# anonymousauthors001/SGS-GNN

Measured on AMD Instinct MI355X. Metric: sampled edges/sec + training steps/sec, Reddit hybrid 20% sparsity, higher is better.
Workload: dtype f32

## Files before the change

include/sgs_hip.h:

```cpp
#ifndef SGS_HIP_H_
#define SGS_HIP_H_

#include <stddef.h>
#include <stdint.h>

#ifdef __cplusplus
extern "C" {
#endif

#define SGS_ABI_VERSION 1

#define SGS_OK 0
#define SGS_EINVAL (-1)
#define SGS_EWORKSPACE (-2)
#define SGS_EHIP (-3)

typedef void* sgs_stream_t;

int sgs_abi_version(void);
const char* sgs_last_error(void);

int sgs_rng_set_epoch_buffer(const uint64_t* epoch_dev);
int sgs_exp_noise(uint64_t seed, uint64_t stream_id, int64_t E, float* noise, sgs_stream_t stream);
int sgs_dropout_keep(uint64_t seed, uint32_t site, int64_t rows, int64_t cols, float p, uint8_t* keep,
// ... 102 lines not shown
                          float* Hn, sgs_stream_t stream);
int sgs_gcn_norm_bwd_edge(const float* gw_hat, const float* gloop, int64_t n_edges, int64_t N, const float* dis,
                          const int32_t* loop_eid, const int64_t* edge_index, const float* Hn, float* dw,
                          sgs_stream_t stream);

#define SGS_ACT_NONE 0
#define SGS_ACT_RELU 1
#define SGS_ACT_RELU_DROPOUT 2
int sgs_spmm_csr(const float* X, int64_t N, int64_t D, int64_t nnz, const int32_t* ptr, const int32_t* col, const float* val,
                 const float* diag, const float* bias, int act, float p_drop, uint64_t seed, uint32_t site, float* Y,
                 sgs_stream_t stream);

int sgs_sddmm_csr(const float* A, const float* B, int64_t N, int64_t D, int64_t nnz, const int32_t* ptr, const int32_t* col,
                  const int32_t* eid, float* g, float* gdiag, sgs_stream_t stream);

int sgs_spmm_csr_variant(int64_t N, int64_t D, int64_t nnz, int aligned16);
int sgs_sddmm_csr_variant(int64_t N, int64_t D, int64_t nnz, int aligned16);

int sgs_act_bwd(const float* dY, const float* Y, int64_t n, int act, float p_drop, float* dZ, sgs_stream_t stream);
size_t sgs_colsum_workspace_bytes(int64_t N, int64_t D);
int sgs_colsum(const float* A, int64_t N, int64_t D, float* out, void* ws, size_t ws_bytes, sgs_stream_t stream);
int sgs_act_bwd_colsum(const float* dY, const float* Y, int64_t N, int64_t D, int act, float p_drop, float* dZ, float* colsum, void* ws,
                       size_t ws_bytes, sgs_stream_t stream);

int sgs_colsum_variant(int64_t N, int64_t D, int fused_act);

int sgs_gcn_pair_ok(int64_t N, int64_t nnz, int64_t D);
int sgs_spmm_csr_next(const float* X, int64_t N, int64_t D, int64_t nnz, const int32_t* ptr, const int32_t* col, const float* val,
                      const float* diag, const float* bias, int act, float p_drop, uint64_t seed, uint32_t site, const float* Wn, int64_t Dn,
                      float* Y, float* Z, sgs_stream_t stream);
int sgs_spmm_csr_bwd_prev(const float* dZ, int64_t N, int64_t D, int64_t nnz, const int32_t* ptr, const int32_t* col, const float* val,
                          const float* diag, const float* W, int64_t Dp, const float* Yp, int act, float p_drop, float* dX, float* dZp,
                          float* colsum, sgs_stream_t stream);

size_t sgs_edge_score_workspace_bytes(int64_t N, int64_t H, int64_t E);
int sgs_edge_score_hidden_supported(int64_t H);
int sgs_edge_score_get_variant(void);
int sgs_edge_score_get_bwd_variant(void);
void sgs_edge_score_set_bwd_variant(int variant);
int sgs_edge_score_bwd_tile(void);
void sgs_edge_score_set_variant(int variant);
int sgs_edge_score_fwd(const float* codes, const float* U, int64_t N, int64_t H, const int64_t* edge_index, int64_t E,
                       int64_t edge_id_offset, const float* W1, const float* b1, const float* w2, const float* b2,
                       float p_drop, uint64_t seed, uint32_t site, float* p_out, void* ws, size_t ws_bytes,
                       sgs_stream_t stream);
size_t sgs_edge_mates_workspace_bytes(int64_t n_edges);
int sgs_edge_mates(const int64_t* edge_index, int64_t n_edges, int64_t N, const int32_t* out_ptr, const int32_t* out_dst,
                   const int32_t* out_eid, int32_t* mate, void* ws, size_t ws_bytes, sgs_stream_t stream);
int sgs_edge_score_paired_supported(int64_t H);
int sgs_edge_score_fwd_paired(const float* codes, const float* U, int64_t N, int64_t H, const int64_t* edge_index, int64_t E,
                              int64_t edge_id_offset, const int32_t* canon, int64_t M, const int32_t* mate, const float* W1, const float* b1,
                              const float* w2, const float* b2, float p_drop, uint64_t seed, uint32_t site, float* p_out, void* ws,
                              size_t ws_bytes, sgs_stream_t stream);
int sgs_edge_score_bwd_core(const float* codes, const float* U, int64_t N, int64_t H, const int64_t* edge_index,
                            int64_t E, int64_t edge_id_offset, const int64_t* active_eid, int64_t n_active, const float* grad_p,
                            const float* W1, const float* b1, const float* w2, const float* b2, float p_drop,
                            uint64_t seed, uint32_t site, float* dv, float* hdz_part, float* dz, float* feat, void* ws,
                            size_t ws_bytes, sgs_stream_t stream);
int sgs_edge_score_bwd_dfeat_supported(int64_t H);
int sgs_edge_score_bwd_dfeat(const float* dv, int64_t n, int64_t H, const float* W1, float* dfeat, void* ws, size_t ws_bytes,
                             sgs_stream_t stream);

int sgs_edge_score_bwd_bits_supported(int64_t H);
int sgs_edge_score_fwd_mask(const float* codes, const float* U, int64_t N, int64_t H, const int64_t* edge_index, int64_t E,
                            int64_t edge_id_offset, const int32_t* canon, int64_t M, const int32_t* mate, const float* W1, const float* b1,
                            const float* w2, const float* b2, float p_drop, uint64_t seed, uint32_t site, float* p_out, uint32_t* maskbits,
// ... 316 lines not shown
```

sgs-gnn_amd/csrc/gcn.hip:

```cpp
#include "sgs_common.h"

namespace sgs {
size_t graph_sort_workspace_bytes(int64_t n, int64_t N);
size_t graph_src_sorted_workspace_bytes(int64_t n, int64_t N);
int graph_build_src_sorted(const int64_t* ei, int64_t n, int64_t N, int32_t* in_ptr, int32_t* in_src, int32_t* in_eid, int32_t* out_ptr,
                           int32_t* out_dst, int32_t* out_eid, int32_t* loop_eid, int32_t* unsorted_flag, void* ws, size_t ws_bytes,
                           hipStream_t stream);
int graph_build_by_sort(const int64_t* ei, int64_t n, int64_t N, int32_t* in_ptr, int32_t* in_src, int32_t* in_eid, int32_t* out_ptr,
                        int32_t* out_dst, int32_t* out_eid, int32_t* loop_eid, void* ws, size_t ws_bytes, hipStream_t stream);
}

namespace sgs {
namespace {

constexpr int kT = 256;
constexpr int kMaxLdsRow = 8192;

__global__ void __launch_bounds__(kT) count_degrees(const int64_t* __restrict__ ei, int64_t n_edges, int* __restrict__ cnt_in,
                                                   int* __restrict__ cnt_out, int* __restrict__ loop_eid) {
    const int64_t e = static_cast<int64_t>(blockIdx.x) * kT + threadIdx.x;
    if (e >= n_edges) return;
    const int s = static_cast<int>(ei[e]), d = static_cast<int>(ei[n_edges + e]);
    atomicAdd(&cnt_in[d], 1);
    atomicAdd(&cnt_out[s], 1);
// ... 968 lines not shown
                                                                 const float* __restrict__ val, const float* __restrict__ diag,
                                                                 const float* __restrict__ bias, int act, float* __restrict__ Y) {
    const int64_t d = blockIdx.y;
    spmm_csr_rowblock_body<VEC, NW>(X + d * xs, N, D, ptr + d * (N + 1), col + d * nnz, val + d * nnz, diag ? diag + d * N : nullptr, bias, act,
                                    1.0f, 0u, uint64_t(0), 0u, nullptr, Y + d * N * D);
}

enum { kPairCol = 0, kPairFwd = 1, kPairBwd = 2 };
constexpr int kPairMaxD = 512;
constexpr int kPairWlds = 12288;
constexpr int kPairWpre = kPairWlds / 1024;
template <class FY, class FW>
__device__ __forceinline__ float lib_gemm_dot(int K, FY y, FW w) {
    const int Kmain = K / 16 * 16;
    float z = 0.f;
    if (Kmain > 0) {
        float ya[8], wa[8];
#pragma unroll
        for (int u = 0; u < 8; ++u) { const int k = 2 * (u & 3) + (u >> 2); ya[u] = y(k); wa[u] = w(k); }
        for (int b = 0; b < Kmain; b += 8) {
            const int nb = b + 8 < Kmain ? b + 8 : b;
            float yn[8], wn[8];
#pragma unroll
            for (int u = 0; u < 8; ++u) { const int k = nb + 2 * (u & 3) + (u >> 2); yn[u] = y(k); wn[u] = w(k); }
#pragma unroll
            for (int u = 0; u < 8; ++u) z = fmaf(ya[u], wa[u], z);
#pragma unroll
            for (int u = 0; u < 8; ++u) { ya[u] = yn[u]; wa[u] = wn[u]; }
        }
    }
    for (int k = Kmain; k < K; ++k) z = fmaf(y(k), w(k), z);
    return z;
}
template <int VEC, int NW, int MODE>
__global__ void __launch_bounds__(1024) spmm_rowgroup_pair(const float* __restrict__ X, int64_t N, int64_t D, const int* __restrict__ ptr,
                                                           const int* __restrict__ col, const float* __restrict__ val,
                                                           const float* __restrict__ diag, const float* __restrict__ bias, int act,
                                                           float drop_scale, uint32_t drop_thresh, uint64_t seed, uint32_t site,
                                                           const uint64_t* __restrict__ epoch, float* __restrict__ Y,
                                                           const float* __restrict__ Wn, int64_t Dn, const float* __restrict__ Yp,
                                                           float* __restrict__ Zn, int ncs, float* __restrict__ colsum) {
    using V = typename VecT<VEC>::type;
    constexpr int RG = 16 / NW;
    __shared__ float part[RG][NW][64 * VEC];
    __shared__ __align__(16) float ys[RG * kPairMaxD];
    __shared__ float wl[MODE == kPairFwd ? kPairWlds : 1];
    if (MODE != kPairFwd && static_cast<int>(blockIdx.x) < ncs) {
        if (D % 4 == 0) colsum_small_v4_body<false>(X, nullptr, N, D, SGS_ACT_NONE, 1.f, nullptr, colsum, blockIdx.x);
        else            colsum_small_body<false>(X, nullptr, N, D, SGS_ACT_NONE, 1.f, nullptr, colsum, blockIdx.x);
        return;
    }
    seed = fold_epoch(seed, epoch);
    const int lane = threadIdx.x & 63, wave = (threadIdx.x >> 6) % NW, grp = threadIdx.x / (64 * NW);
    const int64_t row0 = static_cast<int64_t>(blockIdx.x - ncs) * RG;
    const int64_t i = row0 + grp;
    const bool live = i < N;
    int b = 0, e = 0;
    float dg = 0.f;
    uint32_t rkey = 0;
    const int yact = MODE == kPairBwd ? SGS_ACT_NONE : act;
    if (live) {
        b = ptr[i];
        e = ptr[i + 1];
        dg = diag ? diag[i] : 0.f;
        rkey = dropout_row_key(seed, site, static_cast<uint64_t>(i));
    }
    const bool wlds = MODE == kPairFwd && Dn * D <= kPairWlds;
    float wpre[MODE == kPairFwd ? kPairWpre : 1];
    if (MODE == kPairFwd && wlds) {
#pragma unroll
        for (int u = 0; u < kPairWpre; ++u) {
            const int64_t idx = threadIdx.x + 1024 * u;
            wpre[u] = idx < Dn * D ? Wn[idx] : 0.f;
        }
    }
    for (int64_t cbase = 0; cbase < D; cbase += 64 * VEC) {
        const int64_t c0 = cbase + static_cast<int64_t>(lane) * VEC;
        const bool in = c0 < D;
        float acc[VEC];
#pragma unroll
        for (int v = 0; v < VEC; ++v) acc[v] = 0.f;
        if (in) {
            int k = b + wave;
            for (; k + 7 * NW < e; k += 8 * NW) {
                int j[8]; float w[8]; V x[8];
#pragma unroll
                for (int u = 0; u < 8; ++u) { j[u] = col[k + NW * u]; w[u] = val[k + NW * u]; }
#pragma unroll
                for (int u = 0; u < 8; ++u) x[u] = *reinterpret_cast<const V*>(X + static_cast<int64_t>(j[u]) * D + c0);
#pragma unroll
                for (int u = 0; u < 8; ++u) {
                    float xv[VEC];
                    *reinterpret_cast<V*>(xv) = x[u];
#pragma unroll
                    for (int v = 0; v < VEC; ++v) acc[v] = fmaf(w[u], xv[v], acc[v]);
                }
            }
            for (; k < e; k += NW) {
                float xv[VEC];
                *reinterpret_cast<V*>(xv) = *reinterpret_cast<const V*>(X + static_cast<int64_t>(col[k]) * D + c0);
                const float w = val[k];
#pragma unroll
                for (int v = 0; v < VEC; ++v) acc[v] = fmaf(w, xv[v], acc[v]);
            }
        }
#pragma unroll
        for (int v = 0; v < VEC; ++v) part[grp][wave][lane * VEC + v] = acc[v];
        __syncthreads();
        const int t = threadIdx.x % (64 * NW);
        if (live && t < 64 * VEC && cbase + t < D) {
            const int64_t c = cbase + t;
            float y = 0.f;
#pragma unroll
            for (int g = 0; g < NW; g += 4) y += (part[grp][g][t] + part[grp][g + 1][t]) + (part[grp][g + 2][t] + part[grp][g + 3][t]);
            if (diag) y = fmaf(dg, X[i * D + c], y);
            if (bias) y += bias[c];
            if (yact != SGS_ACT_NONE) y = fmaxf(y, 0.f);
            if (yact == SGS_ACT_RELU_DROPOUT) y = dropout_keep_col(rkey, static_cast<uint32_t>(c), drop_thresh) ? y * drop_scale : 0.f;
            Y[i * D + c] = y;
            ys[grp * D + c] = y;
        }
        __syncthreads();
    }
    if (MODE == kPairFwd) {
        if (wlds) {
#pragma unroll
            for (int u = 0; u < kPairWpre; ++u) {
                const int64_t idx = threadIdx.x + 1024 * u;
                if (idx < Dn * D) {
                    const int64_t o = idx / D, k = idx - o * D;
                    wl[k * Dn + o] = wpre[u];
                }
            }
            __syncthreads();
        }
        for (int64_t idx = threadIdx.x; idx < RG * Dn; idx += 1024) {
            const int r = static_cast<int>(idx / Dn);
            const int64_t o = idx - r * Dn, ir = row0 + r;
            if (ir >= N) break;
            const float* yr = ys + r * D;
            const auto yk = [&](int k) { return yr[k]; };
            Zn[ir * Dn + o] = wlds ? lib_gemm_dot(static_cast<int>(D), yk, [&](int k) { return wl[k * Dn + o]; })
                                   : lib_gemm_dot(static_cast<int>(D), yk, [&](int k) { return Wn[o * D + k]; });
        }
    } else if (MODE == kPairBwd) {
        for (int64_t idx = threadIdx.x; idx < RG * Dn; idx += 1024) {
            const int r = static_cast<int>(idx / Dn);
            const int64_t ep = idx - r * Dn, ir = row0 + r;
            if (ir >= N) break;
            const float* yr = ys + r * D;
            float a = lib_gemm_dot(static_cast<int>(D), [&](int c) { return yr[c]; }, [&](int c) { return Wn[c * Dn + ep]; });
            if (act != SGS_ACT_NONE) a = (Yp[ir * Dn + ep] > 0.f) ? (act == SGS_ACT_RELU_DROPOUT ? a * drop_scale : a) : 0.f;
            Zn[ir * Dn + ep] = a;
        }
    }
}

inline int pick_lpr(int64_t D, int vec) {
    const int64_t need = (D + vec - 1) / vec;
    int lpr = 1;
    while (lpr < need && lpr < 64) lpr <<= 1;
    return lpr;
}

}
}

using namespace sgs;

#define DISPATCH_VEC_LPR(KERNEL, vec, lpr, grid_rows, ...)                                                       \
    do {                                                                                                          \
        const int _rpb = kT / (lpr);                                                                              \
        const dim3 _g(static_cast<unsigned>(cdiv((grid_rows), _rpb))), _b(kT);                                    \
        if ((vec) == 4) {                                                                                         \
            switch (lpr) {                                                                                        \
                case 1: hipLaunchKernelGGL((KERNEL<4, 1>), _g, _b, 0, stream, __VA_ARGS__); break;                \
                case 2: hipLaunchKernelGGL((KERNEL<4, 2>), _g, _b, 0, stream, __VA_ARGS__); break;                \
                case 4: hipLaunchKernelGGL((KERNEL<4, 4>), _g, _b, 0, stream, __VA_ARGS__); break;                \
                case 8: hipLaunchKernelGGL((KERNEL<4, 8>), _g, _b, 0, stream, __VA_ARGS__); break;                \
                case 16: hipLaunchKernelGGL((KERNEL<4, 16>), _g, _b, 0, stream, __VA_ARGS__); break;              \
                case 32: hipLaunchKernelGGL((KERNEL<4, 32>), _g, _b, 0, stream, __VA_ARGS__); break;              \
                default: hipLaunchKernelGGL((KERNEL<4, 64>), _g, _b, 0, stream, __VA_ARGS__); break;              \
            }                                                                                                     \
        } else {                                                                                                  \
            switch (lpr) {                                                                                        \
                case 1: hipLaunchKernelGGL((KERNEL<1, 1>), _g, _b, 0, stream, __VA_ARGS__); break;                \
                case 2: hipLaunchKernelGGL((KERNEL<1, 2>), _g, _b, 0, stream, __VA_ARGS__); break;                \
                case 4: hipLaunchKernelGGL((KERNEL<1, 4>), _g, _b, 0, stream, __VA_ARGS__); break;                \
// ... 486 lines not shown
    PAIR_LAUNCH(kPairFwd, grid, X, N, D, ptr, col, val, diag, bias, act, scale, th, seed, site, epoch_ptr(), Y, Wn, Dn,
                static_cast<const float*>(nullptr), Z, 0, static_cast<float*>(nullptr));
    SGS_LAUNCH_OK();
    return SGS_OK;
}

int sgs_spmm_csr_bwd_prev(const float* dZ, int64_t N, int64_t D, int64_t nnz, const int32_t* ptr, const int32_t* col, const float* val,
                          const float* diag, const float* W, int64_t Dp, const float* Yp, int act, float p_drop, float* dX, float* dZp,
                          float* colsum, sgs_stream_t stream_) {
    hipStream_t stream = static_cast<hipStream_t>(stream_);
    SGS_REQUIRE(sgs_gcn_pair_ok(N, nnz, D), SGS_EINVAL, "sgs_spmm_csr_bwd_prev: not a row-block shape (see sgs_gcn_pair_ok)");
    SGS_REQUIRE(act >= SGS_ACT_NONE && act <= SGS_ACT_RELU_DROPOUT && p_drop >= 0.f && p_drop < 1.f, SGS_EINVAL,
                "sgs_spmm_csr_bwd_prev: bad activation / dropout");
    SGS_REQUIRE(dZ && ptr && dX && dZ != dX, SGS_EINVAL, "sgs_spmm_csr_bwd_prev: null or aliased pointer");
    SGS_REQUIRE(!W || (Dp > 0 && dZp && (act == SGS_ACT_NONE || Yp) && dZp != dX && dZp != dZ), SGS_EINVAL,
                "sgs_spmm_csr_bwd_prev: W needs Dp > 0, dZp and (with an activation) Yp");
    const int vec = (D % 4 == 0 && aligned16(dZ) && aligned16(dX)) ? 4 : 1;
    const bool wide = nnz >= 256 * N;
    const int ncs = colsum ? static_cast<int>(cdiv(D, 16)) : 0;
    const int64_t grid = ncs + cdiv(N, wide ? 1 : 4);
    const float scale = 1.0f / (1.0f - p_drop);
    if (W)
        PAIR_LAUNCH(kPairBwd, grid, dZ, N, D, ptr, col, val, diag, static_cast<const float*>(nullptr), act, scale, 0u, uint64_t(0), 0u,
                    static_cast<const uint64_t*>(nullptr), dX, W, Dp, Yp, dZp, ncs, colsum);
    else
        PAIR_LAUNCH(kPairCol, grid, dZ, N, D, ptr, col, val, diag, static_cast<const float*>(nullptr), SGS_ACT_NONE, 1.f, 0u, uint64_t(0), 0u,
                    static_cast<const uint64_t*>(nullptr), dX, static_cast<const float*>(nullptr), int64_t(0), static_cast<const float*>(nullptr),
                    static_cast<float*>(nullptr), ncs, colsum);
    SGS_LAUNCH_OK();
    return SGS_OK;
}
#undef PAIR_LAUNCH

}

extern "C" {

size_t sgs_graph_filter_multi_workspace_bytes(int64_t E_parent, int64_t N, int64_t D) {
    if (E_parent < 0) E_parent = 0;
    if (N < 0) N = 0;
    if (D < 1) D = 1;
    return 2 * carve_bytes(static_cast<size_t>(D * (N + 1)), 4) + carve_bytes(static_cast<size_t>(D * E_parent + 1), 4) + 256;
}

int sgs_graph_filter_multi(const int32_t* pin_ptr, const int32_t* pin_src, const int32_t* pin_eid, int64_t E_parent, int64_t N, int64_t D,
                           const uint8_t* mask, const int64_t* sampled_eid, int64_t q, int32_t* in_ptr, int32_t* in_src, int32_t* in_eid,
                           int32_t* loop_eid, void* ws, size_t ws_bytes, sgs_stream_t stream_) {
    hipStream_t stream = static_cast<hipStream_t>(stream_);
    SGS_REQUIRE(E_parent >= 0 && N >= 0 && q >= 0 && q <= E_parent && E_parent < (int64_t(1) << 31) && N < (int64_t(1) << 30) && D >= 1 &&
                    D <= 65535, SGS_EINVAL, "sgs_graph_filter_multi: bad sizes");
    if (N == 0) return SGS_OK;
    SGS_REQUIRE(pin_ptr && in_ptr && loop_eid && (E_parent == 0 || (pin_src && pin_eid && mask)) &&
                    (q == 0 || (sampled_eid && in_src && in_eid)), SGS_EINVAL, "sgs_graph_filter_multi: null pointer");
    SGS_REQUIRE(ws && ws_bytes >= sgs_graph_filter_multi_workspace_bytes(E_parent, N, D), SGS_EWORKSPACE,
                "sgs_graph_filter_multi: workspace too small");
    Carver cv(ws);
    int* cnt = cv.take<int>(D * (N + 1));
    int* cur = cv.take<int>(D * (N + 1));
    int* pos = cv.take<int>(D * E_parent + 1);
    const unsigned Du = static_cast<unsigned>(D);
    const int64_t n_row_blocks = cdiv(N * 64, kT);
    const dim3 g1(static_cast<unsigned>(n_row_blocks + cdiv(q, kT)), Du), g3(static_cast<unsigned>(n_row_blocks), Du), blk(kT);
    hipLaunchKernelGGL(multi_filter_count, g1, blk, 0, stream, pin_ptr, pin_eid, N, E_parent, mask, sampled_eid, q, n_row_blocks, cnt, pos);
    if (N <= kSelfScanRows) {
        hipLaunchKernelGGL(multi_filter_fill<true>, g3, blk, 0, stream, pin_ptr, pin_src, pin_eid, N, E_parent, q, mask, pos, in_ptr, in_src, in_eid,
                           loop_eid, static_cast<const int*>(cnt));
// ... 82 lines not shown
```

sgs-gnn_amd/model.py:

```python
from __future__ import annotations

import math

import torch
import torch.nn as nn
import torch.nn.functional as F

from . import ops

SITE_ENC, SITE_SCORE, SITE_GNN, SITE_MLP_X, SITE_MLP_Y = 1, 2, 3, 4, 5


class _DropoutClock:
    base = 0x5D5C0FFEE
    tick = 0

    @classmethod
    def next_seed(cls) -> int:
        cls.tick += 1
        return (cls.base * 0x9E3779B97F4A7C15 + cls.tick * 0xD1B54A32D192ED03) & 0xFFFFFFFFFFFFFFFF


def set_dropout_seed(seed: int) -> None:
    _DropoutClock.base = int(seed) & 0xFFFFFFFFFFFFFFFF
# ... 31 lines not shown
        return y

    def _remember(self, key, x, xl):
        try:
            import weakref
            self._lin_cache = (key, weakref.ref(x), xl)
        except TypeError:
            self._lin_cache = None


class GNNModel(nn.Module):

    def __init__(self, in_channels, hidden_dim, num_classes, dropout_prob=0.3, edge_mlp_type='MLP'):
        super().__init__()
        from .scorer import get_edge_mlp
        self.edge_prob_mlp = get_edge_mlp(in_channels, hidden_dim, dropout_prob, edge_mlp_type)
        self.gcn1 = GCNConv(in_channels, hidden_dim)
        self.dropout = nn.Dropout(dropout_prob)
        self.gcn2 = GCNConv(hidden_dim, num_classes)

    def forward(self, data, edge_index, edge_weight=None):
        from .utils import segment
        x = data.x
        ops.feature_csr(x, build=True)
        with segment(self, "gnn_forward"):
            norm = ops.gcn_norm(ops.get_graph(edge_index, x.shape[0]), edge_weight)
            p = self.dropout.p if self.training else 0.0
            act = ops.ACT_RELU_DROPOUT if p > 0 else ops.ACT_RELU
            xl1, key = self.gcn1._memo(x)
            out, xl1 = ops.gcn2(x, self.gcn1.lin.weight, self.gcn1.bias, self.gcn2.lin.weight, self.gcn2.bias, norm, act=act, p=p,
                                seed=_DropoutClock.next_seed(), site=SITE_GNN, xl1=xl1)
            self.gcn1._remember(key, x, xl1)
            return out


SITE_GAT_ATT, SITE_GAT_ACT = 16, 32


class GATConv(nn.Module):

    def __init__(self, in_channels, out_channels, heads=1, concat=True, negative_slope=0.2, dropout=0.0, edge_dim=None):
        super().__init__()
        heads = int(heads)
        if not 1 <= heads <= 16 or out_channels < 1:
            raise ValueError(f"GATConv: heads = {heads}, out_channels = {out_channels}: 1 <= heads <= 16 and out_channels >= 1 are supported")
        if edge_dim not in (None, 1):
            raise ValueError(f"GATConv: edge_dim = {edge_dim!r}: None and 1 (the edge weight as the attribute) are supported")
        self.in_channels, self.out_channels, self.negative_slope, self.dropout = in_channels, out_channels, negative_slope, dropout
        self.heads, self.concat, self.edge_dim = heads, bool(concat), edge_dim
        self.lin_src = nn.Linear(in_channels, heads * out_channels, bias=False)
        self.lin_dst = self.lin_src
        self.att_src = nn.Parameter(torch.empty(1, heads, out_channels))
        self.att_dst = nn.Parameter(torch.empty(1, heads, out_channels))
        self.bias = nn.Parameter(torch.zeros(heads * out_channels if concat else out_channels))
        a = math.sqrt(6.0 / (in_channels + heads * out_channels))
        nn.init.uniform_(self.lin_src.weight, -a, a)
        b = math.sqrt(6.0 / (heads + out_channels))
        nn.init.uniform_(self.att_src, -b, b)
        nn.init.uniform_(self.att_dst, -b, b)
        if edge_dim is not None:
            self.lin_edge = nn.Linear(edge_dim, heads * out_channels, bias=False)
            self.att_edge = nn.Parameter(torch.empty(1, heads, out_channels))
            e = math.sqrt(6.0 / (edge_dim + heads * out_channels))
            nn.init.uniform_(self.lin_edge.weight, -e, e)
            nn.init.uniform_(self.att_edge, -b, b)

# ... 246 lines not shown
```

sgs-gnn_amd/ops.py:

```python
from __future__ import annotations

import ctypes
import os

import numpy as np
import torch

from . import _lib

SAMPLE_LEARNED, SAMPLE_PRIOR = 0, 1
ACT_NONE, ACT_RELU, ACT_RELU_DROPOUT = 0, 1, 2

_workspaces = {}
_retired_workspaces = []
_pin_workspaces = False


def _need_gpu(*tensors):
    for t in tensors:
        if t is not None and not t.is_cuda:
            raise RuntimeError("sgs_gnn_amd: the SGS hot path runs only on a HIP device (got a CPU tensor); "
                               "there is no CPU fallback")


# ... 1994 lines not shown
            dZ = dY
        need_x, need_W = ctx.needs_input_grad[0], ctx.needs_input_grad[1]
        if need_x or need_W:
            dxl = _spmm(dZ, gr.out_ptr, gr.out_dst, nm.what_out, nm.what_loop, None, ACT_NONE, 0.0, 0, 0, N, D, gr.n_edges)
            if need_W:
                dW = _dyt_x(dxl, x, W.shape, leaf=(ctx, 1))
            if need_x:
                dx = dxl @ W
        if ctx.has_handle and ctx.needs_input_grad[2]:
            g = torch.empty(gr.n_edges + gr.N, dtype=torch.float32, device=dY.device)
            gw, gl = g[:gr.n_edges], g[gr.n_edges:]
            _lib.check(L.sgs_sddmm_csr(_ptr(dZ), _ptr(xl), N, D, gr.n_edges, _ptr(gr.in_ptr), _ptr(gr.in_src), _ptr(gr.in_eid),
                                       gw.data_ptr(), gl.data_ptr(), _stream()), "sgs_sddmm_csr")
        if want_db and dbias is None:
            dbias = _colsum(dZ)
        return dx, dW, (_handle_grad(nm, g) if g is not None else None), dbias, None, None, None, None, None, None


def gcn_layer(x, W, bias, nm: Norm, act=ACT_NONE, p=0.0, seed=0, site=0, xl=None):
    _need_gpu(x, W, bias)
    if x.dtype != torch.float32 or x.dim() != 2 or x.shape[0] != nm.graph.N:
        raise RuntimeError("gcn_layer: x must be float32 [N, F]")
    return _GCNLayer.apply(x, W, nm.handle, bias, nm, act, float(p), int(seed), int(site), xl)


def _pair_ok(gr, *widths):
    L = _lib.lib()
    return all(L.sgs_gcn_pair_ok(gr.N, gr.n_edges, int(w)) for w in widths)


class _GCN2(torch.autograd.Function):

    @staticmethod
    def forward(ctx, x, W1, b1, W2, b2, handle, nm, act, p, seed, site, xl1):
        L = _lib.lib()
        gr = nm.graph
        if xl1 is None:
            xl1 = _x_wt(x, W1)
        N, H = xl1.shape
        C = W2.shape[0]
        fused = _pair_ok(gr, H, C) and xl1.is_contiguous() and W2.is_contiguous() and W2.shape[1] == H
        if fused:
            h = torch.empty(N, H, dtype=torch.float32, device=xl1.device)
            xl2 = torch.empty(N, C, dtype=torch.float32, device=xl1.device)
            _lib.check(L.sgs_spmm_csr_next(_ptr(xl1, torch.float32), N, H, gr.n_edges, _ptr(gr.in_ptr), _ptr(gr.in_src), _ptr(nm.what_in),
                                           _ptr(nm.what_loop), _ptr(b1), act, float(p), seed, site, _ptr(W2, torch.float32), C, _ptr(h),
                                           _ptr(xl2), _stream()), "sgs_spmm_csr_next")
        else:
            h = _spmm(xl1, gr.in_ptr, gr.in_src, nm.what_in, nm.what_loop, b1, act, p, seed, site, N, H, gr.n_edges)
            xl2 = h @ W2.t()
        out = _spmm(xl2, gr.in_ptr, gr.in_src, nm.what_in, nm.what_loop, b2, ACT_NONE, 0.0, 0, 0, N, C, gr.n_edges)
        ctx.nm, ctx.act, ctx.p, ctx.fused = nm, act, p, fused
        ctx.has_b1, ctx.has_b2, ctx.has_handle = b1 is not None, b2 is not None, handle is not None
        ctx.save_for_backward(x, W1, xl1, h, W2, xl2)
        ctx.mark_non_differentiable(xl1)
        ctx.set_materialize_grads(False)
        return out, xl1

    @staticmethod
    def backward(ctx, dout, _dxl_unused):
        L = _lib.lib()
        nm, gr = ctx.nm, ctx.nm.graph
        x, W1, xl1, h, W2, xl2 = ctx.saved_tensors
        N, H = h.shape
        C = W2.shape[0]
        need_x, need_W1, need_b1, need_W2, need_b2, need_g = (ctx.needs_input_grad[i] for i in range(6))
        need_b1, need_b2, need_g = need_b1 and ctx.has_b1, need_b2 and ctx.has_b2, need_g and ctx.has_handle
        dx = dW1 = db1 = dW2 = db2 = g = None
        dZ2 = dout.contiguous()
        f32 = dict(dtype=torch.float32, device=dZ2.device)

        def sddmm(dZ, xl, D):
            gg = torch.empty(gr.n_edges + gr.N, **f32)
            _lib.check(L.sgs_sddmm_csr(_ptr(dZ), _ptr(xl), N, D, gr.n_edges, _ptr(gr.in_ptr), _ptr(gr.in_src), _ptr(gr.in_eid),
                                       gg[:gr.n_edges].data_ptr(), gg[gr.n_edges:].data_ptr(), _stream()), "sgs_sddmm_csr")
            return gg

        want_1 = need_x or need_W1 or need_b1 or need_g
        dxl2 = dZ1 = None
        if want_1 or need_W2:
            dxl2 = torch.empty(N, C, **f32)
            if ctx.fused:
                dZ1 = torch.empty(N, H, **f32) if want_1 else None
                db2 = torch.empty(C, **f32) if need_b2 else None
# ... 3 lines not shown
            else:
                dxl2 = _spmm(dZ2, gr.out_ptr, gr.out_dst, nm.what_out, nm.what_loop, None, ACT_NONE, 0.0, 0, 0, N, C, gr.n_edges)
        if need_W2:
            dW2 = _dyt_x(dxl2, h, W2.shape, leaf=(ctx, 3))
        if want_1 and not ctx.fused:
            dZ1h = dxl2 @ W2
            if need_b1:
                dZ1, db1 = _act_bwd_colsum(dZ1h, h, ctx.act, ctx.p)
            else:
                dZ1 = torch.empty_like(dZ1h)
                _lib.check(L.sgs_act_bwd(_ptr(dZ1h), _ptr(h), dZ1h.numel(), ctx.act, float(ctx.p), _ptr(dZ1), _stream()), "sgs_act_bwd")
        g2 = sddmm(dZ2, xl2, C) if need_g else None
        if need_b2 and db2 is None:
            db2 = _colsum(dZ2)
        if need_x or need_W1 or (need_b1 and db1 is None and ctx.fused):
            if ctx.fused:
                dxl1 = torch.empty(N, H, **f32)
                db1 = torch.empty(H, **f32) if need_b1 else None
                _lib.check(L.sgs_spmm_csr_bwd_prev(_ptr(dZ1), N, H, gr.n_edges, _ptr(gr.out_ptr), _ptr(gr.out_dst), _ptr(nm.what_out),
                                                   _ptr(nm.what_loop), None, 0, None, ACT_NONE, 0.0, _ptr(dxl1), None, _ptr(db1), _stream()),
                           "sgs_spmm_csr_bwd_prev")
            else:
                dxl1 = _spmm(dZ1, gr.out_ptr, gr.out_dst, nm.what_out, nm.what_loop, None, ACT_NONE, 0.0, 0, 0, N, H, gr.n_edges)
            if need_W1:
                dW1 = _dyt_x(dxl1, x, W1.shape, leaf=(ctx, 1))
            if need_x:
                dx = dxl1 @ W1
        g1 = sddmm(dZ1, xl1, H) if need_g else None
        if need_b1 and db1 is None:
            db1 = _colsum(dZ1)
        if need_g:
            r2, r1 = _handle_grad(nm, g2), _handle_grad(nm, g1)
            g = r2 if r1 is None else (r1 if r2 is None else r2 + r1)
        return dx, dW1, db1, dW2, db2, g, None, None, None, None, None, None


def gcn2(x, W1, b1, W2, b2, nm: Norm, act=ACT_RELU, p=0.0, seed=0, site=0, xl1=None):
    _need_gpu(x, W1, b1, W2, b2)
    if x.dtype != torch.float32 or x.dim() != 2 or x.shape[0] != nm.graph.N:
        raise RuntimeError("gcn2: x must be float32 [N, F]")
    return _GCN2.apply(x, W1, b1, W2, b2, nm.handle, nm, act, float(p), int(seed), int(site), xl1)


class MultiSampleResult:
    __slots__ = ("mask", "eid", "edge_index", "stats", "w", "D", "E", "q")


def sample_topq_multi(mode: int, p, prior, c: float, q: int, edge_index, D: int, noise=None, seed: int = 0, stream_id0: int = 0,
                      want_edge_index: bool = True, want_w: bool = False) -> MultiSampleResult:
    L = _lib.lib()
    _need_gpu(p, prior, edge_index, noise)
    if p is None and edge_index is None:
        raise RuntimeError("sample_topq_multi: uniform weights (p=None) need edge_index for the number of candidates")
    E = p.numel() if p is not None else edge_index.shape[1]
    dev = p.device if p is not None else edge_index.device
    D = int(D)
    if noise is not None and (noise.dim() != 2 or tuple(noise.shape) != (D, E)):
        raise RuntimeError(f"sample_topq_multi: noise must be [D={D}, E={E}]")
    r = MultiSampleResult()
    r.D, r.E, r.q = D, E, q
    r.mask = torch.empty(max(D, 1), E, dtype=torch.bool, device=dev)
    r.eid = torch.empty(max(D, 1), q, dtype=torch.int64, device=dev)
    r.edge_index = torch.empty(max(D, 1), 2, q, dtype=torch.int64, device=dev) if (want_edge_index and edge_index is not None) else None
    r.stats = torch.empty(max(D, 1), 4, dtype=torch.float32, device=dev)
    r.w = torch.empty(max(D, 1), q, dtype=torch.float32, device=dev) if want_w else None
    ws = workspace(L.sgs_sample_topq_multi_workspace_bytes(E, max(D, 1)), dev)
    _lib.check(L.sgs_sample_topq_multi(mode, _ptr(p, torch.float32), _ptr(prior, torch.float32), float(c), _ptr(noise, torch.float32), seed,
                                       stream_id0, D, E, q, _ptr(edge_index, torch.int64), _ptr(r.mask), _ptr(r.eid), _ptr(r.edge_index),
                                       _ptr(r.stats), _ptr(r.w), ws.data_ptr(), ws.numel(), _stream()), "sgs_sample_topq_multi")
    return r


def graph_filter_multi(parent: Graph, smp: MultiSampleResult):
    L = _lib.lib()
# ... 447 lines not shown
```

sgs-gnn_amd/training.py:

```python
from __future__ import annotations

import torch
import torch.nn as nn

from . import ops
from .dist import GradSync, is_parallel
from .sampling import cover_graph, cover_nodes, draw_learned, draw_prior, random_edge_sampling
from .utils import segment

_PIPELINES = ("two_pass", "straight_through", "hybrid")


def _fused_ce_ok(criterion) -> bool:
    return (type(criterion) is nn.CrossEntropyLoss and criterion.weight is None and criterion.reduction == "mean"
            and criterion.ignore_index == -100 and getattr(criterion, "label_smoothing", 0.0) == 0.0)


def _ce_spec(criterion):
    if type(criterion) is not nn.CrossEntropyLoss or criterion.reduction != "mean" or criterion.ignore_index != -100:
        return None
    eps = float(getattr(criterion, "label_smoothing", 0.0))
    if not 0.0 <= eps <= 1.0:
        return None
    return criterion.weight, eps
# ... 5 lines not shown
        return ops.masked_cross_entropy(out, batch.y, batch.train_mask, weight=spec[0], label_smoothing=spec[1])
    return criterion(out[batch.train_mask], batch.y[batch.train_mask])


def _backward(model, loss):
    with segment(model, "backward"), ops.deferred_weight_grads(loss):
        loss.backward()


def _has_train_nodes(batch) -> bool:
    flag = getattr(batch, "_sgs_has_train", None)
    if flag is None:
        flag = bool(batch.train_mask.any())
        try:
            batch._sgs_has_train = flag
        except Exception:
            pass
    return flag


class SampledForward:
    __slots__ = ("rsei", "rs", "edge_probs_full", "smp", "sampled_edge_index", "edge_probs_for_loss", "learned_out",
                 "random_out", "cbuf")


def sampled_prefix(args, batch, q, noise=None):
    if not (args.conditional or args.sparse_edge_mlp):
        return None
    noise = noise or {}
    rs = draw_prior(batch.prob, batch.edge_index, q, noise=noise.get("prior"), cover=cover_graph(args, batch))
    graph_r = ops.get_subgraph(batch.edge_index, batch.x.shape[0], rs)
    ops.gcn_norm(graph_r, None)
    return rs


def sampled_forward(pipeline, args, model, batch, q, use_checkpoint=False, noise=None, side_stream=None, prefix=None,
                    gate_publish=None) -> SampledForward:
    noise = noise or {}
    st = SampledForward()
    N = batch.x.shape[0]
    scorer = model.edge_prob_mlp

    st.rsei, st.rs = None, None
    if args.conditional or args.sparse_edge_mlp:
        rs = prefix if prefix is not None else sampled_prefix(args, batch, q, noise)
        st.rsei, st.rs = rs.edge_index, rs
    st.random_out = None
    forked = side_stream is not None and args.conditional and st.rsei is not None
    if forked:
        ops.gcn_norm(ops.get_graph(st.rsei, N), None)
        main_stream = torch.cuda.current_stream()
        side_stream.wait_stream(main_stream)
        with torch.cuda.stream(side_stream), ops.workspace_slot(2):
            ops.workspace_handover(batch.x.device, slot=2)
            st.random_out = model(batch, st.rsei)

    if pipeline == "two_pass":
        with torch.no_grad():
            st.edge_probs_full = scorer(batch.x, batch.edge_index, st.rsei).squeeze()
    elif pipeline == "hybrid":
        st.edge_probs_full = scorer(batch.x, batch.edge_index, st.rsei, use_checkpoint=use_checkpoint).squeeze()
    else:
        st.edge_probs_full = scorer(batch.x, batch.edge_index, st.rsei).squeeze()
    pass1_active = getattr(scorer, "last_active", None)

    st.smp = smp = draw_learned(batch.prob, st.edge_probs_full, batch.edge_index, q, args.degree_bias_coef,
                                noise=noise.get("sample"), want_p=(pipeline == "hybrid"), cover=cover_graph(args, batch))
    st.sampled_edge_index = smp.edge_index
    graph_s = ops.get_subgraph(batch.edge_index, N, smp)

    if pipeline == "hybrid":
        if pass1_active is not None:
            pass1_active.set(smp.eid, graph_s, ascending=True)
        st.edge_probs_for_loss = ops.select_sampled(st.edge_probs_full, smp.eid, smp.p, pass1_active)
    elif pipeline == "straight_through":
        st.edge_probs_for_loss = ops.st_weights(st.edge_probs_full, batch.prob, args.degree_bias_coef, smp.stats, smp.eid)
    else:
        st.edge_probs_for_loss = scorer(batch.x, smp.edge_index).squeeze()
    if forked:
        main_stream.wait_stream(side_stream)
    st.learned_out = model(batch, smp.edge_index, st.edge_probs_for_loss)

    st.cbuf = None
    if args.conditional:
        if st.random_out is None:
            st.random_out = model(batch, st.rsei)
        st.cbuf = ops.gate_counts(st.learned_out, st.random_out, batch.y, batch.train_mask, publish=gate_publish)
    return st


def learned_loss(args, criterion, st: SampledForward, batch):
    c1 = args.regularizer1_coef if args.reg1 == True else 0.0
    c2 = args.consist_reg_coef if args.reg2 == True else 0.0
    spec = _ce_spec(criterion)
    if (c1 != 0.0 or c2 != 0.0) and spec is not None:
        return ops.hybrid_loss(st.learned_out, batch.y, batch.train_mask, st.edge_probs_for_loss, st.sampled_edge_index, c1, c2,
                               weight=spec[0], label_smoothing=spec[1])[0]
    loss = _ce(criterion, st.learned_out, batch)
    if c1 != 0.0 or c2 != 0.0:
        reg, _ = ops.edge_regularizers(st.edge_probs_for_loss, st.learned_out, st.sampled_edge_index, batch.y,
                                       batch.train_mask, c1, c2)
        loss = loss + reg
    return loss


def train(args, epoch, max_epoch, model, optimizer_gnn, optimizer_edge_prob, optimizer, criterion, cluster_loader,
          q=500, alternate_frequency=1):
    pipeline = getattr(args, "pipeline", "two_pass")
    if pipeline not in _PIPELINES:
        pipeline = "two_pass"
    return _train(pipeline, args, epoch, max_epoch, model, optimizer_gnn, optimizer_edge_prob, optimizer, criterion,
                  cluster_loader, q)


# ... 303 lines not shown
```

Baseline: 103.2 million.

## Batch learned and random GCN forward passes into dual-job SpMM kernels

```diff
diff --git a/include/sgs_hip.h b/include/sgs_hip.h
--- a/include/sgs_hip.h
+++ b/include/sgs_hip.h
@@ -158,6 +158,16 @@
 int sgs_spmm_csr_bwd_prev(const float* dZ, int64_t N, int64_t D, int64_t nnz, const int32_t* ptr, const int32_t* col, const float* val,
                           const float* diag, const float* W, int64_t Dp, const float* Yp, int act, float p_drop, float* dX, float* dZp,
                           float* colsum, sgs_stream_t stream);
+
+int sgs_gcn_dual_ok(int64_t N, int64_t nnz_a, int64_t nnz_b, int64_t D, int64_t Dn);
+int sgs_spmm_csr_next_dual(const float* X, int64_t N, int64_t D, const float* bias, int act, float p_drop, uint32_t site, const float* Wn,
+                           int64_t Dn, int64_t nnz_a, const int32_t* ptr_a, const int32_t* col_a, const float* val_a, const float* diag_a,
+                           uint64_t seed_a, float* Y_a, float* Z_a, int64_t nnz_b, const int32_t* ptr_b, const int32_t* col_b,
+                           const float* val_b, const float* diag_b, uint64_t seed_b, float* Y_b, float* Z_b, sgs_stream_t stream);
+int sgs_spmm_csr_dual(const float* X_a, const float* X_b, int64_t N, int64_t D, const float* bias, int act, float p_drop, uint32_t site,
+                      int64_t nnz_a, const int32_t* ptr_a, const int32_t* col_a, const float* val_a, const float* diag_a, uint64_t seed_a,
+                      float* Y_a, int64_t nnz_b, const int32_t* ptr_b, const int32_t* col_b, const float* val_b, const float* diag_b,
+                      uint64_t seed_b, float* Y_b, sgs_stream_t stream);
 
 size_t sgs_edge_score_workspace_bytes(int64_t N, int64_t H, int64_t E);
 int sgs_edge_score_hidden_supported(int64_t H);
diff --git a/sgs-gnn_amd/csrc/gcn.hip b/sgs-gnn_amd/csrc/gcn.hip
--- a/sgs-gnn_amd/csrc/gcn.hip
+++ b/sgs-gnn_amd/csrc/gcn.hip
@@ -1024,14 +1024,14 @@
     for (int k = Kmain; k < K; ++k) z = fmaf(y(k), w(k), z);
     return z;
 }
-template <int VEC, int NW, int MODE>
-__global__ void __launch_bounds__(1024) spmm_rowgroup_pair(const float* __restrict__ X, int64_t N, int64_t D, const int* __restrict__ ptr,
-                                                           const int* __restrict__ col, const float* __restrict__ val,
-                                                           const float* __restrict__ diag, const float* __restrict__ bias, int act,
-                                                           float drop_scale, uint32_t drop_thresh, uint64_t seed, uint32_t site,
-                                                           const uint64_t* __restrict__ epoch, float* __restrict__ Y,
-                                                           const float* __restrict__ Wn, int64_t Dn, const float* __restrict__ Yp,
-                                                           float* __restrict__ Zn, int ncs, float* __restrict__ colsum) {
+template <int VEC, int NW, int MODE, int GU = 8>
+__device__ __forceinline__ void spmm_rowgroup_pair_body(const float* __restrict__ X, int64_t N, int64_t D, const int* __restrict__ ptr,
+                                                        const int* __restrict__ col, const float* __restrict__ val,
+                                                        const float* __restrict__ diag, const float* __restrict__ bias, int act,
+                                                        float drop_scale, uint32_t drop_thresh, uint64_t seed, uint32_t site,
+                                                        const uint64_t* __restrict__ epoch, float* __restrict__ Y,
+                                                        const float* __restrict__ Wn, int64_t Dn, const float* __restrict__ Yp,
+                                                        float* __restrict__ Zn, int ncs, float* __restrict__ colsum) {
     using V = typename VecT<VEC>::type;
     constexpr int RG = 16 / NW;
     __shared__ float part[RG][NW][64 * VEC];
@@ -1074,14 +1074,14 @@
         for (int v = 0; v < VEC; ++v) acc[v] = 0.f;
         if (in) {
             int k = b + wave;
-            for (; k + 7 * NW < e; k += 8 * NW) {
-                int j[8]; float w[8]; V x[8];
-#pragma unroll
-                for (int u = 0; u < 8; ++u) { j[u] = col[k + NW * u]; w[u] = val[k + NW * u]; }
-#pragma unroll
-                for (int u = 0; u < 8; ++u) x[u] = *reinterpret_cast<const V*>(X + static_cast<int64_t>(j[u]) * D + c0);
-#pragma unroll
-                for (int u = 0; u < 8; ++u) {
+            for (; k + (GU - 1) * NW < e; k += GU * NW) {
+                int j[GU]; float w[GU]; V x[GU];
+#pragma unroll
+                for (int u = 0; u < GU; ++u) { j[u] = col[k + NW * u]; w[u] = val[k + NW * u]; }
+#pragma unroll
+                for (int u = 0; u < GU; ++u) x[u] = *reinterpret_cast<const V*>(X + static_cast<int64_t>(j[u]) * D + c0);
+#pragma unroll
+                for (int u = 0; u < GU; ++u) {
                     float xv[VEC];
                     *reinterpret_cast<V*>(xv) = x[u];
 #pragma unroll
@@ -1146,6 +1146,54 @@
             Zn[ir * Dn + ep] = a;
         }
     }
+}
+template <int VEC, int NW, int MODE>
+__global__ void __launch_bounds__(1024) spmm_rowgroup_pair(const float* __restrict__ X, int64_t N, int64_t D, const int* __restrict__ ptr,
+                                                           const int* __restrict__ col, const float* __restrict__ val,
+                                                           const float* __restrict__ diag, const float* __restrict__ bias, int act,
+                                                           float drop_scale, uint32_t drop_thresh, uint64_t seed, uint32_t site,
+                                                           const uint64_t* __restrict__ epoch, float* __restrict__ Y,
+                                                           const float* __restrict__ Wn, int64_t Dn, const float* __restrict__ Yp,
+                                                           float* __restrict__ Zn, int ncs, float* __restrict__ colsum) {
+    spmm_rowgroup_pair_body<VEC, NW, MODE>(X, N, D, ptr, col, val, diag, bias, act, drop_scale, drop_thresh, seed, site, epoch, Y, Wn, Dn, Yp, Zn,
+                                           ncs, colsum);
+}
+
+struct SpmmDualJob {
+    const float* X;
+    const int* ptr;
+    const int* col;
+    const float* val;
+    const float* diag;
+    float* Y;
+    float* Z;
+    int64_t nnz;
+    uint64_t seed;
+};
+struct SpmmDualArgs {
+    SpmmDualJob job[2];
+};
+template <int VEC, int NW>
+__global__ void __launch_bounds__(64 * NW) spmm_csr_rowblock_dual(SpmmDualArgs a, int64_t N, int64_t D, const float* __restrict__ bias, int act,
+                                                                  float drop_scale, uint32_t drop_thresh, uint32_t site,
+                                                                  const uint64_t* __restrict__ epoch) {
+    const SpmmDualJob& j = a.job[blockIdx.y];
+    spmm_csr_rowblock_body<VEC, NW>(j.X, N, D, j.ptr, j.col, j.val, j.diag, bias, act, drop_scale, drop_thresh, j.seed, site, epoch, j.Y);
+}
+#ifndef SGS_DUAL_PAIR_CAPPED
+#define SGS_DUAL_PAIR_CAPPED 1
+#endif
+constexpr int kDualPairWaves = SGS_DUAL_PAIR_CAPPED ? 8 : 4;
+constexpr int dual_pair_gu(int vec) { return SGS_DUAL_PAIR_CAPPED && vec == 4 ? 4 : 8; }
+template <int VEC, int NW>
+__global__ void __launch_bounds__(1024, kDualPairWaves) spmm_rowgroup_pair_dual(SpmmDualArgs a, int64_t N, int64_t D,
+                                                                                const float* __restrict__ bias, int act, float drop_scale,
+                                                                                uint32_t drop_thresh, uint32_t site,
+                                                                                const uint64_t* __restrict__ epoch,
+                                                                                const float* __restrict__ Wn, int64_t Dn) {
+    const SpmmDualJob& j = a.job[blockIdx.y];
+    spmm_rowgroup_pair_body<VEC, NW, kPairFwd, dual_pair_gu(VEC)>(j.X, N, D, j.ptr, j.col, j.val, j.diag, bias, act, drop_scale, drop_thresh, j.seed,
+                                                            site, epoch, j.Y, Wn, Dn, nullptr, j.Z, 0, nullptr);
 }
 
 inline int pick_lpr(int64_t D, int vec) {
@@ -1698,6 +1746,70 @@
 }
 #undef PAIR_LAUNCH
 
+int sgs_gcn_dual_ok(int64_t N, int64_t nnz_a, int64_t nnz_b, int64_t D, int64_t Dn) {
+    return (sgs_gcn_pair_ok(N, nnz_a, D) && sgs_gcn_pair_ok(N, nnz_b, D) && Dn > 0 && (nnz_a >= 256 * N) == (nnz_b >= 256 * N)) ? 1 : 0;
+}
+
+int sgs_spmm_csr_next_dual(const float* X, int64_t N, int64_t D, const float* bias, int act, float p_drop, uint32_t site, const float* Wn,
+                           int64_t Dn, int64_t nnz_a, const int32_t* ptr_a, const int32_t* col_a, const float* val_a, const float* diag_a,
+                           uint64_t seed_a, float* Y_a, float* Z_a, int64_t nnz_b, const int32_t* ptr_b, const int32_t* col_b,
+                           const float* val_b, const float* diag_b, uint64_t seed_b, float* Y_b, float* Z_b, sgs_stream_t stream_) {
+    hipStream_t stream = static_cast<hipStream_t>(stream_);
+    SGS_REQUIRE(sgs_gcn_dual_ok(N, nnz_a, nnz_b, D, Dn), SGS_EINVAL, "sgs_spmm_csr_next_dual: not two row-block shapes of one variant (see sgs_gcn_dual_ok)");
+    SGS_REQUIRE(act >= SGS_ACT_NONE && act <= SGS_ACT_RELU_DROPOUT && p_drop >= 0.f && p_drop < 1.f, SGS_EINVAL,
+                "sgs_spmm_csr_next_dual: bad activation / dropout");
+    SGS_REQUIRE(X && ptr_a && ptr_b && Y_a && Y_b && Wn && Z_a && Z_b && X != Y_a && X != Y_b && X != Z_a && X != Z_b && Y_a != Y_b &&
+                    Z_a != Z_b && Y_a != Z_a && Y_a != Z_b && Y_b != Z_a && Y_b != Z_b,
+                SGS_EINVAL, "sgs_spmm_csr_next_dual: null or aliased pointer");
+    const int vec = (D % 4 == 0 && aligned16(X) && aligned16(Y_a)) ? 4 : 1;
+    SGS_REQUIRE(vec == ((D % 4 == 0 && aligned16(X) && aligned16(Y_b)) ? 4 : 1), SGS_EINVAL,
+                "sgs_spmm_csr_next_dual: the two jobs select different kernel variants (alignment)");
+    const bool wide = nnz_a >= 256 * N;
+    const float scale = 1.0f / (1.0f - p_drop);
+    const uint32_t th = dropout_thresh(p_drop);
+    if (act == SGS_ACT_RELU_DROPOUT && p_drop == 0.f) act = SGS_ACT_RELU;
+    SpmmDualArgs a;
+    a.job[0] = SpmmDualJob{X, ptr_a, col_a, val_a, diag_a, Y_a, Z_a, nnz_a, seed_a};
+    a.job[1] = SpmmDualJob{X, ptr_b, col_b, val_b, diag_b, Y_b, Z_b, nnz_b, seed_b};
+    const dim3 grid(static_cast<unsigned>(cdiv(N, wide ? 1 : 4)), 2);
+    if (vec == 4 && wide)  hipLaunchKernelGGL((spmm_rowgroup_pair_dual<4, 16>), grid, dim3(1024), 0, stream, a, N, D, bias, act, scale, th, site, epoch_ptr(), Wn, Dn);
+    else if (vec == 4)     hipLaunchKernelGGL((spmm_rowgroup_pair_dual<4, 4>), grid, dim3(1024), 0, stream, a, N, D, bias, act, scale, th, site, epoch_ptr(), Wn, Dn);
+    else if (wide)         hipLaunchKernelGGL((spmm_rowgroup_pair_dual<1, 16>), grid, dim3(1024), 0, stream, a, N, D, bias, act, scale, th, site, epoch_ptr(), Wn, Dn);
+    else                   hipLaunchKernelGGL((spmm_rowgroup_pair_dual<1, 4>), grid, dim3(1024), 0, stream, a, N, D, bias, act, scale, th, site, epoch_ptr(), Wn, Dn);
+    SGS_LAUNCH_OK();
+    return SGS_OK;
+}
+
+int sgs_spmm_csr_dual(const float* X_a, const float* X_b, int64_t N, int64_t D, const float* bias, int act, float p_drop, uint32_t site,
+                      int64_t nnz_a, const int32_t* ptr_a, const int32_t* col_a, const float* val_a, const float* diag_a, uint64_t seed_a,
+                      float* Y_a, int64_t nnz_b, const int32_t* ptr_b, const int32_t* col_b, const float* val_b, const float* diag_b,
+                      uint64_t seed_b, float* Y_b, sgs_stream_t stream_) {
+    hipStream_t stream = static_cast<hipStream_t>(stream_);
+    SGS_REQUIRE(N > 0 && D > 0, SGS_EINVAL, "sgs_spmm_csr_dual: bad sizes");
+    SGS_REQUIRE(act >= SGS_ACT_NONE && act <= SGS_ACT_RELU_DROPOUT && p_drop >= 0.f && p_drop < 1.f, SGS_EINVAL,
+                "sgs_spmm_csr_dual: bad activation / dropout");
+    SGS_REQUIRE(X_a && X_b && ptr_a && ptr_b && Y_a && Y_b && Y_a != Y_b && X_a != Y_a && X_a != Y_b && X_b != Y_a && X_b != Y_b, SGS_EINVAL,
+                "sgs_spmm_csr_dual: null or aliased pointer");
+    const int var = sgs_spmm_csr_variant(N, D, nnz_a, aligned16(X_a) && aligned16(Y_a));
+    SGS_REQUIRE(var >= 1000 && var == sgs_spmm_csr_variant(N, D, nnz_b, aligned16(X_b) && aligned16(Y_b)), SGS_EINVAL,
+                "sgs_spmm_csr_dual: not two row-block shapes of one variant (see sgs_spmm_csr_variant)");
+    const float scale = 1.0f / (1.0f - p_drop);
+    const uint32_t th = dropout_thresh(p_drop);
+    if (act == SGS_ACT_RELU_DROPOUT && p_drop == 0.f) act = SGS_ACT_RELU;
+    SpmmDualArgs a;
+    a.job[0] = SpmmDualJob{X_a, ptr_a, col_a, val_a, diag_a, Y_a, nullptr, nnz_a, seed_a};
+    a.job[1] = SpmmDualJob{X_b, ptr_b, col_b, val_b, diag_b, Y_b, nullptr, nnz_b, seed_b};
+    const dim3 g_(static_cast<unsigned>(N), 2);
+    switch (var) {
+        case 1416: hipLaunchKernelGGL((spmm_csr_rowblock_dual<4, 16>), g_, dim3(1024), 0, stream, a, N, D, bias, act, scale, th, site, epoch_ptr()); break;
+        case 1404: hipLaunchKernelGGL((spmm_csr_rowblock_dual<4, 4>), g_, dim3(kT), 0, stream, a, N, D, bias, act, scale, th, site, epoch_ptr()); break;
+        case 1116: hipLaunchKernelGGL((spmm_csr_rowblock_dual<1, 16>), g_, dim3(1024), 0, stream, a, N, D, bias, act, scale, th, site, epoch_ptr()); break;
+        default:   hipLaunchKernelGGL((spmm_csr_rowblock_dual<1, 4>), g_, dim3(kT), 0, stream, a, N, D, bias, act, scale, th, site, epoch_ptr()); break;
+    }
+    SGS_LAUNCH_OK();
+    return SGS_OK;
+}
+
 }
 
 extern "C" {
diff --git a/sgs-gnn_amd/model.py b/sgs-gnn_amd/model.py
--- a/sgs-gnn_amd/model.py
+++ b/sgs-gnn_amd/model.py
@@ -87,6 +87,24 @@
                                 seed=_DropoutClock.next_seed(), site=SITE_GNN, xl1=xl1)
             self.gcn1._remember(key, x, xl1)
             return out
+
+    def forward_pair(self, data, edge_index_a, edge_weight_a, edge_index_b):
+        from .utils import segment
+        x = data.x
+        ops.feature_csr(x, build=True)
+        with segment(self, "gnn_forward"):
+            N = x.shape[0]
+            norm_a = ops.gcn_norm(ops.get_graph(edge_index_a, N), edge_weight_a)
+            norm_b = ops.gcn_norm(ops.get_graph(edge_index_b, N), None)
+            p = self.dropout.p if self.training else 0.0
+            act = ops.ACT_RELU_DROPOUT if p > 0 else ops.ACT_RELU
+            xl1, key = self.gcn1._memo(x)
+            seed_a = _DropoutClock.next_seed()
+            seed_b = _DropoutClock.next_seed()
+            out_a, out_b, xl1 = ops.gcn2_dual(x, self.gcn1.lin.weight, self.gcn1.bias, self.gcn2.lin.weight, self.gcn2.bias, norm_a, norm_b,
+                                              act=act, p=p, seed_a=seed_a, seed_b=seed_b, site=SITE_GNN, xl1=xl1)
+            self.gcn1._remember(key, x, xl1)
+            return out_a, out_b
 
 
 SITE_GAT_ATT, SITE_GAT_ACT = 16, 32
diff --git a/sgs-gnn_amd/ops.py b/sgs-gnn_amd/ops.py
--- a/sgs-gnn_amd/ops.py
+++ b/sgs-gnn_amd/ops.py
@@ -2050,7 +2050,7 @@
 class _GCN2(torch.autograd.Function):
 
     @staticmethod
-    def forward(ctx, x, W1, b1, W2, b2, handle, nm, act, p, seed, site, xl1):
+    def forward(ctx, x, W1, b1, W2, b2, handle, nm, act, p, seed, site, xl1, pre=None):
         L = _lib.lib()
         gr = nm.graph
         if xl1 is None:
@@ -2058,7 +2058,9 @@
         N, H = xl1.shape
         C = W2.shape[0]
         fused = _pair_ok(gr, H, C) and xl1.is_contiguous() and W2.is_contiguous() and W2.shape[1] == H
-        if fused:
+        if pre is not None:
+            h, xl2, out = pre
+        elif fused:
             h = torch.empty(N, H, dtype=torch.float32, device=xl1.device)
             xl2 = torch.empty(N, C, dtype=torch.float32, device=xl1.device)
             _lib.check(L.sgs_spmm_csr_next(_ptr(xl1, torch.float32), N, H, gr.n_edges, _ptr(gr.in_ptr), _ptr(gr.in_src), _ptr(nm.what_in),
@@ -2067,7 +2069,8 @@
         else:
             h = _spmm(xl1, gr.in_ptr, gr.in_src, nm.what_in, nm.what_loop, b1, act, p, seed, site, N, H, gr.n_edges)
             xl2 = h @ W2.t()
-        out = _spmm(xl2, gr.in_ptr, gr.in_src, nm.what_in, nm.what_loop, b2, ACT_NONE, 0.0, 0, 0, N, C, gr.n_edges)
+        if pre is None:
+            out = _spmm(xl2, gr.in_ptr, gr.in_src, nm.what_in, nm.what_loop, b2, ACT_NONE, 0.0, 0, 0, N, C, gr.n_edges)
         ctx.nm, ctx.act, ctx.p, ctx.fused = nm, act, p, fused
         ctx.has_b1, ctx.has_b2, ctx.has_handle = b1 is not None, b2 is not None, handle is not None
         ctx.save_for_backward(x, W1, xl1, h, W2, xl2)
@@ -2137,7 +2140,7 @@
         if need_g:
             r2, r1 = _handle_grad(nm, g2), _handle_grad(nm, g1)
             g = r2 if r1 is None else (r1 if r2 is None else r2 + r1)
-        return dx, dW1, db1, dW2, db2, g, None, None, None, None, None, None
+        return dx, dW1, db1, dW2, db2, g, None, None, None, None, None, None, None
 
 
 def gcn2(x, W1, b1, W2, b2, nm: Norm, act=ACT_RELU, p=0.0, seed=0, site=0, xl1=None):
@@ -2145,6 +2148,64 @@
     if x.dtype != torch.float32 or x.dim() != 2 or x.shape[0] != nm.graph.N:
         raise RuntimeError("gcn2: x must be float32 [N, F]")
     return _GCN2.apply(x, W1, b1, W2, b2, nm.handle, nm, act, float(p), int(seed), int(site), xl1)
+
+
+_gcn_dual_enabled = True
+GCN_DUAL_FORWARDS = {"shared": 0}
+
+
+def set_gcn_dual(on: bool) -> None:
+    global _gcn_dual_enabled
+    _gcn_dual_enabled = bool(on)
+
+
+def gcn_dual_enabled() -> bool:
+    return _gcn_dual_enabled
+
+
+def gcn_dual_ok(gr_a, gr_b, H: int, C: int) -> bool:
+    return (gr_a.N == gr_b.N and bool(_lib.lib().sgs_gcn_dual_ok(gr_a.N, gr_a.n_edges, gr_b.n_edges, int(H), int(C)))
+            and _pair_ok(gr_a, H, C) and _pair_ok(gr_b, H, C))
+
+
+def _gcn2_dual_forward(xl1, b1, W2, b2, nm_a, nm_b, act, p, seed_a, seed_b, site):
+    L = _lib.lib()
+    GCN_DUAL_FORWARDS["shared"] += 1
+    ga, gb = nm_a.graph, nm_b.graph
+    N, H = xl1.shape
+    C = W2.shape[0]
+    f32 = dict(dtype=torch.float32, device=xl1.device)
+    h_a, xl2_a, out_a = torch.empty(N, H, **f32), torch.empty(N, C, **f32), torch.empty(N, C, **f32)
+    h_b, xl2_b, out_b = torch.empty(N, H, **f32), torch.empty(N, C, **f32), torch.empty(N, C, **f32)
+    _lib.check(L.sgs_spmm_csr_next_dual(_ptr(xl1, torch.float32), N, H, _ptr(b1), act, float(p), site, _ptr(W2, torch.float32), C,
+                                        ga.n_edges, _ptr(ga.in_ptr), _ptr(ga.in_src), _ptr(nm_a.what_in), _ptr(nm_a.what_loop), seed_a,
+                                        _ptr(h_a), _ptr(xl2_a),
+                                        gb.n_edges, _ptr(gb.in_ptr), _ptr(gb.in_src), _ptr(nm_b.what_in), _ptr(nm_b.what_loop), seed_b,
+                                        _ptr(h_b), _ptr(xl2_b), _stream()), "sgs_spmm_csr_next_dual")
+    _lib.check(L.sgs_spmm_csr_dual(_ptr(xl2_a), _ptr(xl2_b), N, C, _ptr(b2), ACT_NONE, 0.0, 0,
+                                   ga.n_edges, _ptr(ga.in_ptr), _ptr(ga.in_src), _ptr(nm_a.what_in), _ptr(nm_a.what_loop), 0, _ptr(out_a),
+                                   gb.n_edges, _ptr(gb.in_ptr), _ptr(gb.in_src), _ptr(nm_b.what_in), _ptr(nm_b.what_loop), 0, _ptr(out_b),
+                                   _stream()), "sgs_spmm_csr_dual")
+    return (h_a, xl2_a, out_a), (h_b, xl2_b, out_b)
+
+
+def gcn2_dual(x, W1, b1, W2, b2, nm_a: Norm, nm_b: Norm, act=ACT_RELU, p=0.0, seed_a=0, seed_b=0, site=0, xl1=None):
+    _need_gpu(x, W1, b1, W2, b2)
+    if x.dtype != torch.float32 or x.dim() != 2 or x.shape[0] != nm_a.graph.N or x.shape[0] != nm_b.graph.N:
+        raise RuntimeError("gcn2_dual: x must be float32 [N, F] over both graphs' N nodes")
+    if nm_b.handle is not None:
+        raise RuntimeError("gcn2_dual: branch b takes no edge-weight gradient (nm_b.handle must be None)")
+    H, C = W1.shape[0], W2.shape[0]
+    pre_a = pre_b = None
+    if (_gcn_dual_enabled and gcn_dual_ok(nm_a.graph, nm_b.graph, H, C) and W2.is_contiguous() and W2.shape[1] == H
+            and (xl1 is None or xl1.is_contiguous())):
+        with torch.no_grad():
+            if xl1 is None:
+                xl1 = _x_wt(x, W1).contiguous()
+            pre_a, pre_b = _gcn2_dual_forward(xl1, b1, W2, b2, nm_a, nm_b, act, float(p), int(seed_a), int(seed_b), int(site))
+    out_a, xl1 = _GCN2.apply(x, W1, b1, W2, b2, nm_a.handle, nm_a, act, float(p), int(seed_a), int(site), xl1, pre_a)
+    out_b, xl1 = _GCN2.apply(x, W1, b1, W2, b2, None, nm_b, act, float(p), int(seed_b), int(site), xl1, pre_b)
+    return out_a, out_b, xl1
 
 
 class MultiSampleResult:
diff --git a/sgs-gnn_amd/training.py b/sgs-gnn_amd/training.py
--- a/sgs-gnn_amd/training.py
+++ b/sgs-gnn_amd/training.py
@@ -61,6 +61,16 @@
     graph_r = ops.get_subgraph(batch.edge_index, batch.x.shape[0], rs)
     ops.gcn_norm(graph_r, None)
     return rs
+
+
+def _gcn_dual_applies(args, model, batch, ei_learned, ei_random, forked) -> bool:
+    from .model import GNNModel
+    if not args.conditional or forked or ei_random is None or type(model) is not GNNModel:
+        return False
+    if not (ops.gcn_dual_enabled() and getattr(args, "sgs_gcn_dual", True)):
+        return False
+    N = batch.x.shape[0]
+    return ops.gcn_dual_ok(ops.get_graph(ei_learned, N), ops.get_graph(ei_random, N), model.gcn1.out_channels, model.gcn2.out_channels)
 
 
 def sampled_forward(pipeline, args, model, batch, q, use_checkpoint=False, noise=None, side_stream=None, prefix=None,
@@ -108,7 +118,10 @@
         st.edge_probs_for_loss = scorer(batch.x, smp.edge_index).squeeze()
     if forked:
         main_stream.wait_stream(side_stream)
-    st.learned_out = model(batch, smp.edge_index, st.edge_probs_for_loss)
+    if _gcn_dual_applies(args, model, batch, smp.edge_index, st.rsei, forked):
+        st.learned_out, st.random_out = model.forward_pair(batch, smp.edge_index, st.edge_probs_for_loss, st.rsei)
+    else:
+        st.learned_out = model(batch, smp.edge_index, st.edge_probs_for_loss)
 
     st.cbuf = None
     if args.conditional:
```

Result: faster. 105.5 million (median of 6 runs) (+2.2%).
